# annappo/GPS-SDR-Receiver

Hardware: AMD Instinct MI355X
Metric: IQ Msamples/s ingested, 32-SV acq + 12-ch track (higher is better)
Workload: dtype f32

## Files before the change

### gps-sdr-receiver_amd/csrc/gpsmi_fft.h

```cpp
#pragma once
#include <hip/hip_runtime.h>

namespace gpsmi {

__device__ __forceinline__ void lds_barrier() {
    asm volatile("s_waitcnt lgkmcnt(0)\n\ts_barrier" ::: "memory");
}


constexpr int kFftN = 2048;
constexpr int kFftThreads = 256;
constexpr int kFftPlane = kFftN + kFftN / 32;
constexpr int kFftPlane1 = kFftN + 8 * (kFftN / 64);
constexpr int kFftLdsFloats = 2 * kFftPlane + 2 * kFftPlane1;

__device__ __forceinline__ int fft_pad(int i) { return i + (i >> 5); }
__device__ __forceinline__ int fft_pad1(int i) { return i + 8 * (i >> 6); }

typedef float fft_c __attribute__((ext_vector_type(2)));

__device__ __forceinline__ fft_c cadd_mi(fft_c a, fft_c b) {
    fft_c d;
    asm("v_pk_add_f32 %0, %1, %2 op_sel:[0,1] op_sel_hi:[1,0] neg_hi:[0,1]" : "=v"(d) : "v"(a), "v"(b));
    return d;
}
__device__ __forceinline__ fft_c cadd_pi(fft_c a, fft_c b) {
    fft_c d;
    asm("v_pk_add_f32 %0, %1, %2 op_sel:[0,1] op_sel_hi:[1,0] neg_lo:[0,1]" : "=v"(d) : "v"(a), "v"(b));
    return d;
}
__device__ __forceinline__ fft_c cneg_add_mi(fft_c a) {
    fft_c d;
    asm("v_pk_add_f32 %0, %1, %1 op_sel:[0,1] op_sel_hi:[1,0] neg_lo:[1,0] neg_hi:[1,1]" : "=v"(d) : "v"(a));
    return d;
}
__device__ __forceinline__ fft_c cmulp(fft_c a, fft_c w) {
    fft_c d;
    asm("v_pk_mul_f32 %0, %2, %1 op_sel_hi:[1,0]\n\t"
        "v_pk_fma_f32 %0, %2, %1, %0 op_sel:[1,1,0] op_sel_hi:[0,1,1] neg_lo:[1,0,0]"
        : "=&v"(d) : "v"(a), "v"(w));
    return d;
}

__device__ __forceinline__ fft_c cmulp_conj(fft_c a, fft_c w) {
    fft_c d;
    asm("v_pk_mul_f32 %0, %2, %1 op_sel_hi:[1,0]\n\t"
        "v_pk_fma_f32 %0, %2, %1, %0 op_sel:[1,1,0] op_sel_hi:[0,1,1] neg_hi:[1,0,0]"
        : "=&v"(d) : "v"(a), "v"(w));
    return d;
}

template <bool B2MI>
__device__ __forceinline__ void dft4p(fft_c& b0, fft_c& b1, fft_c& b2, fft_c& b3) {
    const fft_c c0 = B2MI ? cadd_mi(b0, b2) : b0 + b2;
    const fft_c c1 = B2MI ? cadd_pi(b0, b2) : b0 - b2;
    const fft_c c2 = b1 + b3, d = b1 - b3;
    b0 = c0 + c2;
    b2 = c0 - c2;
    b1 = cadd_mi(c1, d);
    b3 = cadd_pi(c1, d);
}

__device__ __forceinline__ void dft8p(fft_c* v) {
    const float h = 0.70710678118654752440f;
    fft_c a0 = v[0] + v[4], a4 = v[0] - v[4];
    fft_c a1 = v[1] + v[5], a5 = v[1] - v[5];
    fft_c a2 = v[2] + v[6], a6 = v[2] - v[6];
    fft_c a3 = v[3] + v[7], a7 = v[3] - v[7];
    a5 = cadd_mi(a5, a5) * h;
    a7 = cneg_add_mi(a7) * h;
    dft4p<false>(a0, a1, a2, a3);
    dft4p<true>(a4, a5, a6, a7);
    v[0] = a0; v[2] = a1; v[4] = a2; v[6] = a3;
    v[1] = a4; v[3] = a5; v[5] = a6; v[7] = a7;
}

constexpr int kFftTwFloats = 2 * (64 + 512);
struct FftTw {
    const fft_c* t64;
    const fft_c* t512;
    fft_c w4[2][3];
};

__device__ __forceinline__ FftTw fft_setup(float* lds_tw, const float2* __restrict__ tw, int t) {
    float2* t64 = reinterpret_cast<float2*>(lds_tw);
    float2* t512 = t64 + 64;
    t64[t & 63] = tw[32 * (t & 63)];
    t512[t] = tw[4 * t];
    t512[t + 256] = tw[4 * (t + 256)];
    FftTw f;
    f.t64 = reinterpret_cast<const fft_c*>(t64);
    f.t512 = reinterpret_cast<const fft_c*>(t512);
#pragma unroll
    for (int b = 0; b < 2; ++b)
#pragma unroll
        for (int r = 1; r <= 3; ++r) {
            const float2 w = tw[r * (t + 256 * b)];
            f.w4[b][r - 1] = fft_c{w.x, w.y};
        }
    return f;
}

__device__ __forceinline__ void fft2048(float2* vio, float* lds, const FftTw& tw, int t) {
    fft_c* buf0 = reinterpret_cast<fft_c*>(lds);
    fft_c* buf1 = buf0 + kFftPlane;
    fft_c v[8];
#pragma unroll
    for (int r = 0; r < 8; ++r) v[r] = fft_c{vio[r].x, vio[r].y};

    dft8p(v);
#pragma unroll
    for (int r = 0; r < 8; ++r) buf0[fft_pad(8 * t + r)] = v[r];
    lds_barrier();
#pragma unroll
    for (int r = 0; r < 8; ++r) v[r] = buf0[fft_pad(t + 256 * r)];
    {
        const int k = t & 7;
#pragma unroll
        for (int r = 1; r < 8; ++r) v[r] = cmulp(v[r], tw.t64[r * k]);
        dft8p(v);
        const int base = (t >> 3) * 64 + k;
#pragma unroll
        for (int r = 0; r < 8; ++r) buf1[fft_pad1(base + 8 * r)] = v[r];
    }
    lds_barrier();
#pragma unroll
    for (int r = 0; r < 8; ++r) v[r] = buf1[fft_pad1(t + 256 * r)];
    {
        const int k = t & 63;
#pragma unroll
        for (int r = 1; r < 8; ++r) v[r] = cmulp(v[r], tw.t512[r * k]);
        dft8p(v);
        const int base = (t >> 6) * 512 + k;
#pragma unroll
        for (int r = 0; r < 8; ++r) buf0[fft_pad(base + 64 * r)] = v[r];
    }
    lds_barrier();
#pragma unroll
    for (int r = 0; r < 8; ++r) v[r] = buf0[fft_pad(t + 256 * r)];
#pragma unroll
    for (int b = 0; b < 2; ++b) {
        fft_c z1 = cmulp(v[b + 2], tw.w4[b][0]);
        fft_c z2 = cmulp(v[b + 4], tw.w4[b][1]);
        fft_c z3 = cmulp(v[b + 6], tw.w4[b][2]);
        fft_c z0 = v[b];
        dft4p<false>(z0, z1, z2, z3);
        v[b] = z0; v[b + 2] = z1; v[b + 4] = z2; v[b + 6] = z3;
    }
#pragma unroll
    for (int r = 0; r < 8; ++r) vio[r] = make_float2(v[r].x, v[r].y);
}

}
```

### gps-sdr-receiver_amd/csrc/gpsmi_trk_corr.h

```cpp
#pragma once
#include <type_traits>
#include "gpsmi_fft.h"
#include "gpsmi_stats.h"
#include "gpsmi_wgmap.h"

namespace gpsmi {

template <int CG> constexpr int kFoldDepthOf = CG == 1 ? 8 : 3;
constexpr int kFoldChunk = 8;

struct CorrFin { int bi; float bv, mean, sd, elo, ehi; };

__device__ __forceinline__ void corr_finish(const StreamChan& s, const CorrFin& f, const TrkParams& P,
                                            const int* __restrict__ delay_forced,
                                            gpsmi_trk_out* __restrict__ out, JobMid* __restrict__ mid) {
    const int bi = f.bi;
    const float bv = f.bv, mean = f.mean, sd = f.sd, elo = f.elo, ehi = f.ehi;
    const float norm = (bv - mean) / sd;
    gpsmi_trk_out& o = out[s.job];
    o.prn = s.prn;
    o.mx = bi;
    o.epl[0] = elo; o.epl[1] = bv; o.epl[2] = ehi;
    o.corr_mean = mean; o.corr_std = sd;
    o.norm_max_corr = norm;
    int delay = -1;
    double cp = -1.0;
    if (norm > P.corr_min) {
        delay = bi;
        cp = fit_code_phase((double)elo, (double)bv, (double)ehi, bi);
    }
    o.delay = delay;
    o.reserved0 = 0;
    o.code_phase = cp;
    int used = delay >= 0 ? delay : s.d;
    if (delay_forced && delay_forced[s.job] >= 0) used = delay_forced[s.job];
    o.delay_used = used;
    JobMid md;
    md.delay_used = used; md.active = 1; md.prn = s.prn; md.om = s.om; md.ph = s.ph;
    md.pad[0] = md.pad[1] = md.pad[2] = 0;
    mid[s.job] = md;
}

template <int CG, int FMT = 0>
__global__ __launch_bounds__(256, (CG > 4 || CG == 1) ? 2 : 3) void trk_corr_kernel(
    const void* __restrict__ iq, const gpsmi_trk_state* __restrict__ st_in,
    const int* __restrict__ delay_forced, const float2* __restrict__ rep,
    const float2* __restrict__ tw, TrkParams P, int ngroups, int nblocks,
    gpsmi_trk_out* __restrict__ out, JobMid* __restrict__ mid) {
    __shared__ __attribute__((aligned(16))) float lds[kFftLdsFloats];
    __shared__ __attribute__((aligned(16))) float lds_tw[kFftTwFloats];
    __shared__ float red[kStatsRedFloats];
    float* magbuf = lds + 2 * kFftPlane;
    float2 (*urow)[32] = reinterpret_cast<float2 (*)[32]>(lds + 2 * kFftPlane);
    float2 (*vtab)[32] = urow + CG;
    float2* step = reinterpret_cast<float2*>(urow + 2 * CG);
    static_assert(kFftN <= 2 * kFftPlane1 && (CG * 64 + CG) * 2 <= 2 * kFftPlane1, "aliases must fit buffer 1");
    __shared__ StreamChan schan[CG];
    __shared__ CorrFin fin[CG];

    const CorrWg unit = corr_wg_map((int)blockIdx.x, nblocks, ngroups);
    const int g = unit.group, b = unit.block;
    if (b >= nblocks) return;
    const int t = threadIdx.x;
    const int cs = kFftN;
    constexpr int kFoldDepth = kFoldDepthOf<CG>;
    const float2* blk = static_cast<const float2*>(iq) + (size_t)b * ((size_t)cs * P.n_cyc);
    const uint16_t* rblk = static_cast<const uint16_t*>(iq) + (size_t)b * ((size_t)cs * P.n_cyc);
    const double inv_2pi = 0.15915494309189533576888376337251;
    const int first = (P.n_cyc - P.corr_avg) / 2;
    const int pc_c = min(t / 33, CG - 1);
    const gpsmi_trk_state& st = st_in[b * P.nch + min(g * CG + pc_c, P.nch - 1)];
    int st_prn = st.prn, st_delay = st.delay;
    float st_om0 = st.omega0, st_freq = st.freq, st_phase = st.phase;
    using Raw = typename std::conditional<FMT == 0, v2f, unsigned>::type;
    auto fetch = [&](int i, int r) -> Raw {
        if constexpr (FMT == 0) {
            const float2 v = blk[(size_t)i * cs + t + 256 * r];
            return v2f{v.x, v.y};
        } else {
            return (unsigned)rblk[(size_t)i * cs + t + 256 * r];
        }
    };
    auto decode = [&](Raw v) -> v2f {
        if constexpr (FMT == 0) {
            return v;
        } else {
            const float scl = 1.0f / 127.5f;
            return v2f{sub_rn(mul_rn((float)(v & 0xFF), scl), 1.0f), sub_rn(mul_rn((float)(v >> 8), scl), 1.0f)};
        }
    };
    Raw x[kFoldDepth][8];
    const bool nofold = diag_flag(P, 32);
    const bool piped = P.corr_avg == kFoldChunk && !nofold;
    if (piped) {
#pragma unroll
        for (int k = 0; k < kFoldDepth; ++k)
#pragma unroll
            for (int r = 0; r < 8; ++r) x[k][r] = fetch(first + k, r);
    }
    const FftTw ftw = fft_setup(lds_tw, tw, t);
    asm volatile("" : "+v"(st_prn), "+v"(st_delay), "+v"(st_om0), "+v"(st_freq), "+v"(st_phase));

    if (t < CG * 33) {
        const int c = t / 33, i = t % 33;
        const int cidx = g * CG + c;
        const int job = b * P.nch + cidx;
        StreamChan s;
        s.job = job; s.active = 0; s.om = 0.f; s.ph = 0.f; s.d = 0; s.prn = 0;
        if (cidx < P.nch && st_prn > 0) {
            s.active = 1;
            s.om = st_om0 != 0.f ? st_om0 : omega_of(st_freq);
            s.ph = st_phase;
            s.d = st_delay;
            s.prn = st_prn;
        }
        const double f_eff = (double)s.om * inv_2pi;
        if (i < 32) {
            const double rev = f_eff * (double)i * 1.0e-3;
            urow[c][i] = phasor_rev((float)(rev - rint(rev)));
            const double per = f_eff / (1000.0 * (double)cs);
            const double rv = i < 16 ? per * (double)(i + 1) + (double)s.ph * inv_2pi
                                     : per * (double)(16 * (i - 16));
            vtab[c][i] = phasor_rev((float)(rv - rint(rv)));
        } else {
            const double rev = f_eff * 256.0 / (1000.0 * (double)cs);
            step[c] = phasor_rev((float)(rev - rint(rev)));
            schan[c] = s;
            if (cidx < P.nch && !s.active) {
                JobMid z;
                z.delay_used = 0; z.active = 0; z.prn = 0; z.om = 0.f; z.ph = 0.f;
                z.pad[0] = z.pad[1] = z.pad[2] = 0;
                mid[job] = z;
            }
        }
    }
    lds_barrier();

    v2f acc[CG][8];
#pragma unroll
    for (int c = 0; c < CG; ++c)
#pragma unroll
        for (int r = 0; r < 8; ++r) acc[c][r] = v2f{0.f, 0.f};
    auto fold_in = [&](const v2f (&u)[CG], int r, v2f xr, v2f xprev) {
        if constexpr (CG == 1) {
            if (r & 1) cmac2(acc[0][r - 1], acc[0][r], u[0], xprev, u[0], xr);
        } else {
#pragma unroll
            for (int c = 0; c + 1 < CG; c += 2)
                cmac2(acc[c][r], acc[c + 1][r], u[c], xr, u[c + 1], xr);
        }
    };
    auto fold_row = [&](int i, Raw (&xk)[8], auto reload, int inext) {
        v2f u[CG];
#pragma unroll
        for (int c = 0; c < CG; ++c) u[c] = v2f{urow[c][i].x, urow[c][i].y};
        v2f xprev = v2f{0.f, 0.f};
#pragma unroll
        for (int r = 0; r < 8; ++r) {
            const v2f xr = decode(xk[r]);
            fold_in(u, r, xr, xprev);
            xprev = xr;
            if constexpr (decltype(reload)::value) {
                if (CG > 1 || (r & 1)) {
                    xk[r] = fetch(inext, r);
                    if (CG == 1) xk[r - 1] = fetch(inext, r - 1);
                }
            }
        }
    };
    if (piped) {
#pragma unroll
        for (int j = 0; j < kFoldChunk; ++j) {
            if (j + kFoldDepth < kFoldChunk)
                fold_row(first + j, x[j % kFoldDepth], std::true_type{}, first + j + kFoldDepth);
            else
                fold_row(first + j, x[j % kFoldDepth], std::false_type{}, 0);
            __builtin_amdgcn_sched_barrier(0);
        }
    } else if (!nofold) {
        for (int i = first; i < first + P.corr_avg; ++i) {
#pragma unroll
            for (int r = 0; r < 8; ++r) x[0][r] = fetch(i, r);
            fold_row(i, x[0], std::false_type{}, 0);
        }
    }

    const float sc = (1.0f / (float)P.corr_avg) * (1.0f / kFftN);
#pragma unroll
    for (int c = 0; c < CG; ++c) {
        const float2 e1 = vtab[c][t & 15], e2 = vtab[c][16 + (t >> 4)], s2 = step[c];
        fft_c vm = cmulp(fft_c{e1.x, e1.y}, fft_c{e2.x, e2.y});
        const fft_c st256 = fft_c{s2.x, s2.y};
#pragma unroll
        for (int r = 0; r < 8; ++r) {
            acc[c][r] = cmulp(acc[c][r] * sc, vm);
            vm = cmulp(vm, st256);
        }
    }
    auto prepare = [&](int c, const StreamChan& s, float2 (&v)[8], float2 (&rs)[8]) {
#pragma unroll
        for (int r = 0; r < 8; ++r) v[r] = make_float2(acc[c][r].x, acc[c][r].y);
        const float2* R = rep + (size_t)s.prn * kFftN;
#pragma unroll
        for (int q = 0; q < 8; ++q) rs[q] = R[t + 256 * q];
    };
    auto times_conj = [&](float2 (&v)[8], const float2 (&rs)[8]) {
#pragma unroll
        for (int q = 0; q < 8; ++q) {
            const fft_c o = cmulp_conj(fft_c{v[q].x, v[q].y}, fft_c{rs[q].x, rs[q].y});
            v[q] = make_float2(o.x, o.y);
        }
    };
    auto magnitudes = [&](const float2 (&v)[8], float (&mag)[8]) {
#pragma unroll
        for (int q = 0; q < 8; ++q)
            mag[q] = __builtin_amdgcn_sqrtf(v[q].x * v[q].x + v[q].y * v[q].y);
    };
    auto single = [&](int c) {
        const StreamChan s = schan[c];
        float2 v[8], rs[8];
        prepare(c, s, v, rs);
        fft2048(v, lds, ftw, t);
        times_conj(v, rs);
        lds_barrier();
        fft2048(v, lds, ftw, t);
        float mag[8];
        magnitudes(v, mag);
        int bi; float bv, mean, sd, elo, ehi;
        corr_stats8(mag, t, magbuf, red, bi, bv, mean, sd, elo, ehi);
        if (t == 0) fin[c] = CorrFin{bi, bv, mean, sd, elo, ehi};
    };
    if (diag_flag(P, 64)) {
        float sm = 0.f;
#pragma unroll
        for (int c = 0; c < CG; ++c)
#pragma unroll
            for (int r = 0; r < 8; ++r) sm += acc[c][r].x + acc[c][r].y;
        if (t < CG && schan[t].active)
            corr_finish(schan[t], CorrFin{0, sm, 0.f, 1.f, 0.f, 0.f}, P, delay_forced, out, mid);
        return;
    }
#pragma unroll
    for (int c = 0; c < CG; ++c)
        if (schan[c].active) single(c);
    __syncthreads();
    if (t < CG && schan[t].active) corr_finish(schan[t], fin[t], P, delay_forced, out, mid);
}

}
```

Before: 292,200.

## Cut register pressure in CG=4 tracking correlator and hoist FFT LDS index math

For the CG=4 correlator variant, this lowers fold prefetch depth from 3 to 2 and defers loading the radix-4 twiddles until after the fold loop. It also moves the replica loads to after the first FFT, and caps waves per EU at 3, so the variant can hold more registers without spilling. Separately, the FFT now computes its padded LDS indices once per thread and adds constant strides instead of recomputing the pad function per element. The cost is less latency hiding during the fold and on replica fetches for CG=4, since those loads now sit closer to their first use.

```diff
diff --git a/gps-sdr-receiver_amd/csrc/gpsmi_fft.h b/gps-sdr-receiver_amd/csrc/gpsmi_fft.h
--- a/gps-sdr-receiver_amd/csrc/gpsmi_fft.h
+++ b/gps-sdr-receiver_amd/csrc/gpsmi_fft.h
@@ -82,6 +82,16 @@
     fft_c w4[2][3];
 };
 
+__device__ __forceinline__ void fft_setup_w4(FftTw& f, const float2* __restrict__ tw, int t) {
+#pragma unroll
+    for (int b = 0; b < 2; ++b)
+#pragma unroll
+        for (int r = 1; r <= 3; ++r) {
+            const float2 w = tw[r * (t + 256 * b)];
+            f.w4[b][r - 1] = fft_c{w.x, w.y};
+        }
+}
+template <bool W4 = true>
 __device__ __forceinline__ FftTw fft_setup(float* lds_tw, const float2* __restrict__ tw, int t) {
     float2* t64 = reinterpret_cast<float2*>(lds_tw);
     float2* t512 = t64 + 64;
@@ -91,13 +101,7 @@
     FftTw f;
     f.t64 = reinterpret_cast<const fft_c*>(t64);
     f.t512 = reinterpret_cast<const fft_c*>(t512);
-#pragma unroll
-    for (int b = 0; b < 2; ++b)
-#pragma unroll
-        for (int r = 1; r <= 3; ++r) {
-            const float2 w = tw[r * (t + 256 * b)];
-            f.w4[b][r - 1] = fft_c{w.x, w.y};
-        }
+    if constexpr (W4) fft_setup_w4(f, tw, t);
     return f;
 }
 
@@ -108,36 +112,40 @@
 #pragma unroll
     for (int r = 0; r < 8; ++r) v[r] = fft_c{vio[r].x, vio[r].y};
 
+    const int g0 = fft_pad(t), g1 = fft_pad1(t);
     dft8p(v);
+    {
+        const int base = fft_pad(8 * t);
 #pragma unroll
-    for (int r = 0; r < 8; ++r) buf0[fft_pad(8 * t + r)] = v[r];
+        for (int r = 0; r < 8; ++r) buf0[base + r] = v[r];
+    }
     lds_barrier();
 #pragma unroll
-    for (int r = 0; r < 8; ++r) v[r] = buf0[fft_pad(t + 256 * r)];
+    for (int r = 0; r < 8; ++r) v[r] = buf0[g0 + 264 * r];
     {
         const int k = t & 7;
 #pragma unroll
         for (int r = 1; r < 8; ++r) v[r] = cmulp(v[r], tw.t64[r * k]);
         dft8p(v);
-        const int base = (t >> 3) * 64 + k;
+        const int base = fft_pad1((t >> 3) * 64 + k);
 #pragma unroll
-        for (int r = 0; r < 8; ++r) buf1[fft_pad1(base + 8 * r)] = v[r];
+        for (int r = 0; r < 8; ++r) buf1[base + 8 * r] = v[r];
     }
     lds_barrier();
 #pragma unroll
-    for (int r = 0; r < 8; ++r) v[r] = buf1[fft_pad1(t + 256 * r)];
+    for (int r = 0; r < 8; ++r) v[r] = buf1[g1 + 288 * r];
     {
         const int k = t & 63;
 #pragma unroll
         for (int r = 1; r < 8; ++r) v[r] = cmulp(v[r], tw.t512[r * k]);
         dft8p(v);
-        const int base = (t >> 6) * 512 + k;
+        const int base = fft_pad((t >> 6) * 512 + k);
 #pragma unroll
-        for (int r = 0; r < 8; ++r) buf0[fft_pad(base + 64 * r)] = v[r];
+        for (int r = 0; r < 8; ++r) buf0[base + 66 * r] = v[r];
     }
     lds_barrier();
 #pragma unroll
-    for (int r = 0; r < 8; ++r) v[r] = buf0[fft_pad(t + 256 * r)];
+    for (int r = 0; r < 8; ++r) v[r] = buf0[g0 + 264 * r];
 #pragma unroll
     for (int b = 0; b < 2; ++b) {
         fft_c z1 = cmulp(v[b + 2], tw.w4[b][0]);
diff --git a/gps-sdr-receiver_amd/csrc/gpsmi_trk_corr.h b/gps-sdr-receiver_amd/csrc/gpsmi_trk_corr.h
--- a/gps-sdr-receiver_amd/csrc/gpsmi_trk_corr.h
+++ b/gps-sdr-receiver_amd/csrc/gpsmi_trk_corr.h
@@ -6,7 +6,7 @@
 
 namespace gpsmi {
 
-template <int CG> constexpr int kFoldDepthOf = CG == 1 ? 8 : 3;
+template <int CG> constexpr int kFoldDepthOf = CG == 1 ? 8 : CG == 4 ? 2 : 3;
 constexpr int kFoldChunk = 8;
 
 struct CorrFin { int bi; float bv, mean, sd, elo, ehi; };
@@ -42,7 +42,8 @@
 }
 
 template <int CG, int FMT = 0>
-__global__ __launch_bounds__(256, (CG > 4 || CG == 1) ? 2 : 3) void trk_corr_kernel(
+__global__ __launch_bounds__(256)
+__attribute__((amdgpu_waves_per_eu((CG > 4 || CG == 1) ? 2 : 3, CG == 4 ? 3 : 8))) void trk_corr_kernel(
     const void* __restrict__ iq, const gpsmi_trk_state* __restrict__ st_in,
     const int* __restrict__ delay_forced, const float2* __restrict__ rep,
     const float2* __restrict__ tw, TrkParams P, int ngroups, int nblocks,
@@ -64,6 +65,7 @@
     const int t = threadIdx.x;
     const int cs = kFftN;
     constexpr int kFoldDepth = kFoldDepthOf<CG>;
+    constexpr bool kLean = CG == 4;
     const float2* blk = static_cast<const float2*>(iq) + (size_t)b * ((size_t)cs * P.n_cyc);
     const uint16_t* rblk = static_cast<const uint16_t*>(iq) + (size_t)b * ((size_t)cs * P.n_cyc);
     const double inv_2pi = 0.15915494309189533576888376337251;
@@ -98,7 +100,7 @@
 #pragma unroll
             for (int r = 0; r < 8; ++r) x[k][r] = fetch(first + k, r);
     }
-    const FftTw ftw = fft_setup(lds_tw, tw, t);
+    FftTw ftw = fft_setup<!kLean>(lds_tw, tw, t);
     asm volatile("" : "+v"(st_prn), "+v"(st_delay), "+v"(st_om0), "+v"(st_freq), "+v"(st_phase));
 
     if (t < CG * 33) {
@@ -185,6 +187,7 @@
         }
     }
 
+    if constexpr (kLean) fft_setup_w4(ftw, tw, t);
     const float sc = (1.0f / (float)P.corr_avg) * (1.0f / kFftN);
 #pragma unroll
     for (int c = 0; c < CG; ++c) {
@@ -197,9 +200,11 @@
             vm = cmulp(vm, st256);
         }
     }
-    auto prepare = [&](int c, const StreamChan& s, float2 (&v)[8], float2 (&rs)[8]) {
+    auto prepare = [&](int c, float2 (&v)[8]) {
 #pragma unroll
         for (int r = 0; r < 8; ++r) v[r] = make_float2(acc[c][r].x, acc[c][r].y);
+    };
+    auto replica = [&](const StreamChan& s, float2 (&rs)[8]) {
         const float2* R = rep + (size_t)s.prn * kFftN;
 #pragma unroll
         for (int q = 0; q < 8; ++q) rs[q] = R[t + 256 * q];
@@ -219,8 +224,10 @@
     auto single = [&](int c) {
         const StreamChan s = schan[c];
         float2 v[8], rs[8];
-        prepare(c, s, v, rs);
+        prepare(c, v);
+        if constexpr (!kLean) replica(s, rs);
         fft2048(v, lds, ftw, t);
+        if constexpr (kLean) replica(s, rs);
         times_conj(v, rs);
         lds_barrier();
         fft2048(v, lds, ftw, t);
```

Result: faster. 299,200 (median of 6 runs) (+2.4%).
